# aask1357/hilcodec

Hardware: AMD Instinct MI355X
Metric: audio-seconds/sec (xRT) encode+RVQ+decode, 24 kHz batch=256 (higher is better)
Workload: dtype f32

## Files before the change

hilcodec_amd/csrc/resblock_kernel.h:

```cpp
#pragma once
#include "resblock_gemm.h"
#include "stream_gemm.h"

namespace {

struct Cols {
  long b;
  int t;
  int t_in;
  unsigned boff;
  unsigned hoff;
  int head, tail;
};
static_assert(sizeof(Cols) == 32, "no padding");

template <int C, bool STREAM, bool SCARRY = false, int NB = 1, bool W8 = false, int DRU = 0, bool POST = false, bool SPEC0 = false>
__global__ __launch_bounds__((Cfg<C, STREAM, SCARRY, NB, W8, DRU, POST, SPEC0>::NT), (Cfg<C, STREAM, SCARRY, NB, W8, DRU, POST, SPEC0>::MINW)) void resblock_kernel(ResArgs a) {
  using K = Cfg<C, STREAM, SCARRY, NB, W8, DRU, POST, SPEC0>;
  constexpr int DR = K::DR, UR = K::UR;
  using Pipe = WeightPipe<K>;
  constexpr int CBW = K::CBW, NW = K::NW, NT = K::NT, RW = K::RW, RB = K::RB, XS = K::XS, TO = K::TO, RSTEP = K::RSTEP;
  __shared__ __attribute__((aligned(16))) float Xbuf[4 + C * XS];
  constexpr bool DW_RELOAD = NB > 1 && K::NARROW && (4 + C * XS + NB * C * DWS) * 4 > 156 * 1024;
  __shared__ __attribute__((aligned(16))) float DW[(DW_RELOAD ? 1 : NB) * C * DWS];
  constexpr bool DWIDE = DR == 5 || DR == 8;
  __shared__ __attribute__((aligned(16))) float DWD[(DR > 0 && !DWIDE) ? 2 * C * DDS : 4];
  __shared__ __attribute__((aligned(16))) float HS[(STREAM && !K::NARROW) ? 2 * C * 4 : 4];
  __shared__ __attribute__((aligned(16))) float PR[POST ? POST_CLASSES * K::NCOL : 4];
  static_assert(!POST || (K::RPI * K::NW == POST_CLASSES), "a row class of the closing conv = the rows one half-wave walks");
  __shared__ __attribute__((aligned(16))) float SEG[SPEC0 ? (STREAM ? 256 : 192) : 4];
  __shared__ __attribute__((aligned(16))) float SEGS[SPEC0 ? (STREAM ? 256 : 192) : 4];
  float* const X = Xbuf + 4;
  const int tid = threadIdx.x, lane = tid & 63;
  const int wave = __builtin_amdgcn_readfirstlane(tid >> 6);
  constexpr int NCB = K::NCOL / 32;
  const int colblk = wave % NCB;
  const int wclass = wave / NCB;
  const int rowblk0 = wclass * CBW;
#if defined(HILC_DEBUG_WAVE_STAMPS)
  constexpr int WS_MAXB = 48;
  unsigned long long* ws_base = nullptr;
  int ws_k = 0;
#define STAMP(i) do { } while (0)
#define lds_barrier() do {                                                                                          \
    const unsigned long long t0_ = __builtin_amdgcn_s_memtime();                                                   \
    asm volatile("s_waitcnt lgkmcnt(0)" ::: "memory");                                                             \
    const unsigned long long t1_ = __builtin_amdgcn_s_memtime();                                                   \
    asm volatile("s_waitcnt lgkmcnt(0)\n\ts_barrier" ::: "memory");                                                 \
    const unsigned long long t2_ = __builtin_amdgcn_s_memtime();                                                   \
    if (ws_base != nullptr && lane == 0 && ws_k < WS_MAXB - 1) {                                                   \
      ws_base[ws_k * 3] = t0_; ws_base[ws_k * 3 + 1] = t1_; ws_base[ws_k * 3 + 2] = t2_;                           \
    }                                                                                                              \
    ++ws_k;                                                                                                        \
  } while (0)
#elif defined(HILC_DEBUG_STAMPS)
#define STAMP(i) do { if (a.dbg && tid == 0) a.dbg[stamp_tile * 8 + (i)] = __builtin_amdgcn_s_memtime(); } while (0)
  long stamp_tile = blockIdx.x;
#else
#define STAMP(i) do { } while (0)
#endif
  const int T = a.T;
  const int nblk = NB == 1 ? 1 : a.nblk;
  auto load_taps = [&](const ResBlk& bq, float* dst) {
    if constexpr (DW_RELOAD && !STREAM) {
      constexpr int NE = C * DWS;
      static_assert(NE % NT == 0, "whole rounds");
#pragma unroll
      for (int i = 0; i < NE / NT; ++i) {
        const int e = tid + i * NT;
        const int m = e / DWS, j = e - m * DWS;
        const float* src = j < 5 ? bq.dw1_w + (m * 5 + j) : (j == 5 ? bq.dw1_b + m : (j < 11 ? bq.dw2_w + (m * 5 + (j - 6)) : bq.dw2_b + m));
        dst[e] = *src;
      }
    } else if constexpr (DW_RELOAD) {
      constexpr int NE = C * DWS;
      static_assert(NE % NT == 0, "whole rounds");
#pragma unroll 3
      for (int i = 0; i < NE / NT; ++i) {
        const int e = tid + i * NT;
        const int m = e / DWS, j = e - m * DWS;
        const float* src = j < 5 ? bq.dw1_w + (m * 5 + j) : (j == 5 ? bq.dw1_b + m : (j < 11 ? bq.dw2_w + (m * 5 + (j - 6)) : bq.dw2_b + m));
        dst[e] = *src;
      }
    }
  };
  if constexpr (!DW_RELOAD) {
    constexpr int RND = (C + NT - 1) / NT;
    if constexpr (NB == 1 && STREAM) {
      const ResBlk& bq = a.blk[0];
#pragma unroll
      for (int it = 0; it < RND; ++it) {
        const int m = tid + it * NT;
        const int mc = (C % NT == 0 || m < C) ? m : C - 1;
#pragma unroll
        for (int w4 = 0; w4 < DWS / 4; ++w4) {
          float t4[4];
#pragma unroll
          for (int e = 0; e < 4; ++e) {
            const int j = 4 * w4 + e;
            t4[e] = j < 5 ? bq.dw1_w[mc * 5 + j] : (j == 5 ? bq.dw1_b[mc] : (j < 11 ? bq.dw2_w[mc * 5 + (j - 6)] : bq.dw2_b[mc]));
          }
          if (C % NT == 0 || m < C) *reinterpret_cast<f32x4*>(&DW[m * DWS + 4 * w4]) = f32x4{t4[0], t4[1], t4[2], t4[3]};
          __builtin_amdgcn_sched_barrier(0);
        }
      }
    } else {
    float tv[NB][RND][DWS];
#pragma unroll
    for (int q = 0; q < NB; ++q) {
      if (q < nblk) {
        const ResBlk& bq = a.blk[q];
#pragma unroll
        for (int it = 0; it < RND; ++it) {
          const int m = tid + it * NT;
          const int mc = (C % NT == 0 || m < C) ? m : C - 1;
#pragma unroll
          for (int j = 0; j < 5; ++j) tv[q][it][j] = bq.dw1_w[mc * 5 + j];
          tv[q][it][5] = bq.dw1_b[mc];
#pragma unroll
          for (int j = 0; j < 5; ++j) tv[q][it][6 + j] = bq.dw2_w[mc * 5 + j];
          tv[q][it][11] = bq.dw2_b[mc];
        }
      }
    }
#pragma unroll
    for (int q = 0; q < NB; ++q) {
      if (q < nblk) {
#pragma unroll
        for (int it = 0; it < RND; ++it) {
          const int m = tid + it * NT;
          if (C % NT == 0 || m < C) {
#pragma unroll
            for (int w4 = 0; w4 < DWS / 4; ++w4)
              *reinterpret_cast<f32x4*>(&DW[(q * C + m) * DWS + 4 * w4]) =
                  f32x4{tv[q][it][4 * w4], tv[q][it][4 * w4 + 1], tv[q][it][4 * w4 + 2], tv[q][it][4 * w4 + 3]};
          }
        }
      }
    }
    }
  }
  if constexpr (DR > 0 && !DWIDE) {
    constexpr int RND = (2 * C + NT - 1) / NT;
    float tw[RND][2 * DR + 1];
#pragma unroll
    for (int it = 0; it < RND; ++it) {
      const int m = tid + it * NT;
      const int mc = ((2 * C) % NT == 0 || m < 2 * C) ? m : 2 * C - 1;
#pragma unroll
      for (int j = 0; j < 2 * DR; ++j) tw[it][j] = a.dn.dw_w[mc * 2 * DR + j];
      tw[it][2 * DR] = a.dn.dw_b[mc];
    }
#pragma unroll
    for (int it = 0; it < RND; ++it) {
      const int m = tid + it * NT;
      if ((2 * C) % NT == 0 || m < 2 * C) {
#pragma unroll
        for (int j = 0; j < DDS; ++j) DWD[m * DDS + j] = j < 2 * DR ? tw[it][j] : (j == 8 ? tw[it][2 * DR] : 0.f);
      }
    }
  }
  if (tid < 4) Xbuf[tid] = 0.f;
  const int rsub = wave * K::RPI + (K::RPI > 1 ? lane / (K::NCOL / 4) : 0);
  const int c4 = (lane & (K::NCOL / 4 - 1)) * 4;
  [[maybe_unused]] const unsigned row_b = (unsigned)T * 4u;
  [[maybe_unused]] const bool one_head = STREAM && !K::NARROW && T >= K::NCOL;

  auto columns_of = [&](long tile) -> Cols {
    Cols s;
    s.boff = 0; s.hoff = 0; s.head = false; s.tail = false;
    if constexpr (STREAM) {
      const int flat = (int)tile * TO - K::HALO + c4;
      s.t_in = flat >= 0 && flat < a.B * T;
      const unsigned ub = s.t_in ? __umulhi((unsigned)flat, a.div_magic) >> a.div_shift : 0u;
      s.b = ub;
      s.t = s.t_in ? flat - (int)ub * T : 0;
      s.boff = (ub * (unsigned)(C * T) + (unsigned)s.t) * 4u;
      s.hoff = ub * (unsigned)(C * 4);
      s.head = s.t_in && s.t == 0;
      s.tail = s.t_in && c4 >= K::HALO && s.t == T - 4;
    } else {
      s.b = tile / a.tiles;
      s.t = (int)(tile - s.b * a.tiles) * TO + c4;
      s.t_in = s.t >= 0 && s.t < T;
    }
    return s;
  };
  auto xrow = [&](const Cols& s, int m) -> const f32x4* {
    if constexpr (STREAM)
      return reinterpret_cast<const f32x4*>(reinterpret_cast<const char*>(a.x) + (s.boff + (unsigned)m * row_b));
    else
      return reinterpret_cast<const f32x4*>(a.x + s.b * (long)C * T + (long)m * T + (s.t_in ? s.t : 0));
  };
  auto yrow = [&](const Cols& s, int m) -> f32x4* {
    if constexpr (STREAM)
      return reinterpret_cast<f32x4*>(reinterpret_cast<char*>(a.y) + (s.boff + (unsigned)m * row_b));
    else
      return reinterpret_cast<f32x4*>(a.y + s.b * (long)C * T + (long)m * T + s.t);
  };

  [[maybe_unused]] const float* hb0 = a.x;
  [[maybe_unused]] const float* hb1 = a.x;
  [[maybe_unused]] bool hv0 = false, hv1 = false;
  [[maybe_unused]] int blk_off = 0;
  Cols cs;
  const bool lane0 = c4 == 0, lane_last = c4 == K::NCOL - 4;
  auto prev_base = [&](int which) -> lptr_t {
    if constexpr (!K::CARRYMODE) return (lptr_t)(X + rsub * XS + c4 - 4);
    else return lane0 ? (lptr_t)(X + rsub * XS + K::NCOL + which * 4 + blk_off) : (lptr_t)(X + rsub * XS + c4 - 4);
  };
  auto prevs_of = [&](lptr_t pb, int m0, int which, f32x4 (&prev)[K::RB]) {
    if constexpr (!STREAM) {
#pragma unroll
      for (int i = 0; i < K::RB; ++i) prev[i] = *(lvec_t)(pb + i * RSTEP * XS);
    } else {
      bool staged = false;
      if constexpr (!K::NARROW) staged = one_head;
      if (staged) {
#pragma unroll
        for (int i = 0; i < K::RB; ++i) {
          const lptr_t pa = cs.head ? (lptr_t)(HS + (which * C + m0 + RSTEP * i) * 4) : pb + i * RSTEP * XS;
          prev[i] = *(lvec_t)pa;
        }
      } else {
        f32x4 hv[K::RB];
#pragma unroll
        for (int i = 0; i < K::RB; ++i)
          hv[i] = *reinterpret_cast<const f32x4*>((which ? hb1 : hb0) + ((which ? hv1 : hv0) ? cs.hoff + (unsigned)(m0 + RSTEP * i) * 4u : 0u));
#pragma unroll
        for (int i = 0; i < K::RB; ++i) {
          const f32x4 own = *(lvec_t)(pb + i * RSTEP * XS);
#pragma unroll
          for (int e = 0; e < 4; ++e) prev[i][e] = cs.head ? ((which ? hv1 : hv0) ? hv[i][e] : 0.f) : own[e];
        }
      }
    }
  };
  auto carry_out = [&](lptr_t xp, int which, const f32x4 (&cur)[K::RB]) {
    if constexpr (K::CARRYMODE) {
      if (lane_last) {
#pragma unroll
        for (int i = 0; i < K::RB; ++i) *(lvec_t)(xp + i * RSTEP * XS + 4 + which * 4 + blk_off) = cur[i];
      }
    }
  };

  float touch = 0.f;
  constexpr int LPR = K::NCOL / 32;
#ifdef HILC_RES_NO_UTOUCH
  constexpr bool UTOUCH = false;
#else
  constexpr bool UTOUCH = !STREAM && UR > 0 && !K::NARROW && (K::NCOL / (UR > 0 ? UR : 1)) % 32 == 0;
#endif
  constexpr int LPRU = UTOUCH ? K::NCOL / UR / 32 : 1;
  constexpr int NTOUCH = STREAM ? 1 : (UTOUCH ? (2 * C * LPRU + NT - 1) / NT : (C * LPR + NT - 1) / NT);
  float tv[NTOUCH];
#pragma unroll
  for (int i = 0; i < NTOUCH; ++i) tv[i] = 0.f;
  __shared__ long s_next;
  long run0 = blockIdx.x, run1 = a.total_tiles;
  long tile = blockIdx.x;
  if constexpr (K::CARRYMODE) {
    if (a.classes > 1) {
      const unsigned P = gridDim.x / (unsigned)a.classes, u = blockIdx.x % P, c = blockIdx.x / P;
      const long s0 = (long)u * a.total_tiles / P, len = (long)(u + 1) * a.total_tiles / P - s0;
      run0 = s0 + ((len * (long)a.cum[c]) >> 16);
      run1 = s0 + ((len * (long)a.cum[c + 1]) >> 16);
    } else if (a.run_tiles > 0) {
      run0 = (long)blockIdx.x * a.run_tiles;
      run1 = run0 + a.run_tiles < a.total_tiles ? run0 + a.run_tiles : a.total_tiles;
    } else {
      run0 = (long)blockIdx.x * a.total_tiles / gridDim.x;
      run1 = ((long)blockIdx.x + 1) * a.total_tiles / gridDim.x;
    }
    const bool mid = STREAM ? (run0 * TO) % T != 0 : run0 % a.tiles != 0;
    tile = (mid && run0 < run1) ? run0 - 1 : run0;
  }
  cs = columns_of(tile < run1 ? tile : 0);
  f32x4 xr[RW];
  if (UR == 0 && !SPEC0 && tile < run1) {
#pragma unroll
    for (int i = 0; i < RW; ++i) xr[i] = *xrow(cs, rsub + RSTEP * i);
  }
// ... 54 lines not shown
              const long row = (long)cs.b * (2 * C) + k;
              const float* xi = up.xin + (cs.t_in ? row * Tin + q0 : 0);
              xc[i] = xi[0];
              const float* pp = has_prev ? xi - 1 : (up.hist != nullptr && cs.t_in ? up.hist + row : xi);
              xq[i] = pp[0];
              if constexpr (UR == 2) {
                xn[i] = xi[cs.t_in ? 1 : 0];
                wa[i] = *reinterpret_cast<const f32x4*>(up.tr_w + k * 4);
              } else if constexpr (UEXP) {
                xn[i] = xi[has_next ? 1 : 0];
                const float* tw = up.tr_w + ((long)k * UR + p0) * 8;
                wa[i] = *reinterpret_cast<const f32x4*>(tw);
                wb[i] = *reinterpret_cast<const f32x4*>(tw + 4);
              } else {
                wa[i] = *reinterpret_cast<const f32x4*>(up.tr_w + k * (2 * UR) + p0);
                wb[i] = *reinterpret_cast<const f32x4*>(up.tr_w + k * (2 * UR) + UR + p0);
              }
            }
#pragma unroll
            for (int i = 0; i < UB; ++i) {
              const float a1 = prologue(xc[i], up.in_scale, 1);
              const float a0 = has_prev ? prologue(xq[i], up.in_scale, 1) : (up.hist != nullptr ? xq[i] : 0.f);
              f32x4 u;
              float a_last = a1;
              if constexpr (UR == 2) {
                const float a2 = prologue(xn[i], up.in_scale, 1);
                u[0] = fmaf(wa[i].x, a1, wa[i].z * a0);
                u[1] = fmaf(wa[i].y, a1, wa[i].w * a0);
                u[2] = fmaf(wa[i].x, a2, wa[i].z * a1);
                u[3] = fmaf(wa[i].y, a2, wa[i].w * a1);
                a_last = a2;
              } else if constexpr (UEXP) {
                const float a2 = has_next ? prologue(xn[i], up.in_scale, 1) : 0.f;
#pragma unroll
                for (int e = 0; e < 4; ++e) {
                  const bool nx = p0 + e >= UR;
                  u[e] = fmaf(wa[i][e], nx ? a2 : a1, wb[i][e] * (nx ? a1 : a0));
                }
                a_last = p0 + 3 >= UR ? a2 : a1;
              } else {
#pragma unroll
                for (int e = 0; e < 4; ++e) u[e] = fmaf(wa[i][e], a1, wb[i][e] * a0);
              }
              *(lvec_t)(xp + i * RSTEP * XS) = zero_unless(cs.t_in, u);
              if constexpr (STREAM) {
                if (cs.tail && !warm && up.hist_out != nullptr)
                  up.hist_out[(long)cs.b * (2 * C) + h * C + rsub + RSTEP * (i0 + i)] = a_last;
              }
            }
            xp += UB * RSTEP * XS;
            asm volatile("" : "+v"(xp));
            __builtin_amdgcn_sched_barrier(0);
          }
        }
        Pipe wp;
        wp.prefetch(wu, lane);
        lds_barrier();
        if constexpr (K::NARROW) gemm_phase_rolled<K, false>(wu, X, acc, wp, colblk, lane);
        else gemm_phase<K, false>(wu, X, acc, wp, colblk, lane);
        lds_barrier();
      }
      acc_to_x<K>(acc, X, rowblk0, colblk, lane);
      lds_barrier();
      {
        lptr_t xp = (lptr_t)(X + rsub * XS + c4);
#pragma unroll
        for (int i = 0; i < RW; ++i) {
          const float bv = up.bias != nullptr ? up.bias[rsub + RSTEP * i] : 0.f;
          f32x4 v = *(lvec_t)(xp + i * RSTEP * XS);
#pragma unroll
          for (int e = 0; e < 4; ++e) v[e] = up.bias != nullptr ? __fadd_rn(v[e], bv) : v[e];
          xr[i] = v;
        }
      }
      lds_barrier();
    }
    if constexpr (SPEC0) {
      const ResSpec0& sp = a.spec;
      constexpr int N = 64, NBIN = 33, SROWS = 40, KP0 = 4, DEPTH0 = 2;
      [[maybe_unused]] int split = K::NCOL;
      if constexpr (STREAM) {
        const int F0 = (int)tile * TO;
        const unsigned bA = __umulhi((unsigned)F0, a.div_magic) >> a.div_shift;
        const int tA0 = F0 - (int)bA * T;
        const int nxt = T - tA0;
        split = nxt < K::NCOL ? nxt : K::NCOL;
        const int lenA = (N - 1) + split;
        for (int i = tid; i < 2 * (N - 1) + K::NCOL; i += NT) {
          const bool second = i >= lenA;
          const unsigned b = bA + (second ? 1u : 0u);
          const int t = second ? i - lenA - (N - 1) : tA0 - (N - 1) + i;
          float v = 0.f;
          if (b < (unsigned)a.B) {
            if (t >= 0) v = sp.wav[(long)b * T + t];
            else if (sp.hist != nullptr && t >= -sp.hist_len) v = sp.hist[(long)b * sp.hist_len + sp.hist_len + t];
          }
          SEG[i] = v;
          SEGS[i] = v * sp.pre_in_scale;
        }
        for (int i = tid; i < (SROWS - NBIN) * 128; i += NT) X[(NBIN + (i >> 7)) * XS + (i & 127)] = 0.f;
      } else {
      const int f0 = cs.t - c4;
      {
        const int s0 = f0 - (N - 1);
        const float* wb = sp.wav + cs.b * (long)T;
        for (int i = tid; i < 127 + N; i += NT) {
          const int t = s0 + i;
          const float v = (t >= 0 && t < T) ? wb[t] : 0.f;
          SEG[i] = v;
          SEGS[i] = v * sp.pre_in_scale;
        }
        for (int i = tid; i < (SROWS - NBIN) * 128; i += NT) X[(NBIN + (i >> 7)) * XS + (i & 127)] = 0.f;
      }
      }
      lds_barrier();
      const int kh = lane >> 5, col = colblk * 32 + (lane & 31);
      const int colx = col + ((STREAM && col >= split) ? N - 1 : 0);
      f32x16 acc[CBW];
      {
        int off[8];
#pragma unroll
        for (int p = 0; p < 8; ++p) off[p] = colx + 2 * p + kh;
        auto bop = [&](int P) -> float { return SEG[off[P & 7] + 16 * (P >> 3)]; };
        stream_gemm<CBW, KP0, DEPTH0, N / 2 / KP0>(sp.dft, acc, lane, bop);
      }
      float nyq_im = 0.f;
#pragma unroll 8
      for (int k = 0; k < N; ++k) nyq_im = fmaf(sp.nyq[k], SEG[colx + k], nyq_im);
      const SpecFinish finish = SpecFinish::make(sp.mean, sp.stdv, sp.normalize);
#pragma unroll
      for (int i = 0; i < CBW; ++i) {
#pragma unroll
        for (int r = 0; r < 16; r += 2) {
          const int row = i * 32 + acc_row(r, lane);
          if (i == 0 && r == 0) {
            if (kh == 0) {
              X[0 * XS + col] = finish(acc[0][0], 0.f);
              X[(N / 2) * XS + col] = finish(acc[0][1], nyq_im);
            } else {
              X[(row >> 1) * XS + col] = finish(acc[0][0], acc[0][1]);
            }
          } else {
            X[(row >> 1) * XS + col] = finish(acc[i][r], acc[i][r + 1]);
          }
        }
      }
      lds_barrier();
      {
        const float* sl = X + kh * XS + col;
        auto bop = [&](int P) -> float { return sl[2 * P * XS]; };
        stream_gemm<CBW, KP0, DEPTH0, SROWS / 2 / KP0>(sp.pw, acc, lane, bop);
      }
      lds_barrier();
      acc_to_x<K>(acc, X, rowblk0, colblk, lane);
      lds_barrier();
      {
        lptr_t xp = (lptr_t)(X + rsub * XS + c4);
        float sm[8];
        const int c4x = c4 + ((STREAM && c4 >= split) ? N - 1 : 0);
#pragma unroll
        for (int j = 0; j < 8; ++j) sm[j] = SEGS[c4x + j + N - 5];
#pragma unroll
        for (int i = 0; i < RW; ++i) {
          const int m = rsub + RSTEP * i;
          const float bv = sp.bias != nullptr ? sp.bias[m] : 0.f;
          const float pb = sp.pre_b != nullptr ? sp.pre_b[m] : 0.f;
          float w5[5];
#pragma unroll
          for (int j = 0; j < 5; ++j) w5[j] = sp.pre_w[m * 5 + j];
          f32x4 v = *(lvec_t)(xp + i * RSTEP * XS);
#pragma unroll
          for (int e = 0; e < 4; ++e) {
            float acc5 = 0.f;
#pragma unroll
            for (int j = 0; j < 5; ++j) acc5 = fmaf(w5[j], sm[e + j], acc5);
            const float rr = sp.pre_b != nullptr ? __fadd_rn(acc5, pb) : acc5;
            float t = v[e];
            if (sp.bias != nullptr) t = __fadd_rn(t, bv);
            t = __fmul_rn(t, sp.out_scale);
            v[e] = __fadd_rn(t, rr);
          }
          xr[i] = v;
          if (i % 2 == 1) __builtin_amdgcn_sched_barrier(0);
        }
      }
      lds_barrier();
    }
#pragma nounroll
    for (int blk = 0; blk < nblk; ++blk) {
    const ResBlk& bp = a.blk[NB == 1 ? 0 : blk];
    const bool final_blk = NB == 1 || blk == nblk - 1;
    const bool last_blk = DR == 0 && !POST && final_blk;
    [[maybe_unused]] const bool post_blk = POST && final_blk;
    Cols cn = cs;
    bool have_next = false;
    if constexpr (NB > 1) blk_off = 8 * blk;
    const float* const DWb = DW + ((NB == 1 || DW_RELOAD) ? 0 : blk * C * DWS);
    if constexpr (DW_RELOAD) load_taps(bp, DW);
    if constexpr (STREAM) {
      hb0 = bp.hist1 != nullptr ? bp.hist1 : a.x;
      hb1 = bp.hist2 != nullptr ? bp.hist2 : a.x;
      hv0 = bp.hist1 != nullptr;
      hv1 = bp.hist2 != nullptr;
    }
    const float* w1t = bp.w1t + (long)wclass * (C * C / K::RH);
    const float* w2t = bp.w2t + (long)wclass * (C * C / K::RH);
    asm volatile("" : "+s"(w1t), "+s"(w2t));
    [[maybe_unused]] f32x4 hstage[(STREAM && !K::NARROW) ? (2 * C + NT - 1) / NT : 1];
    [[maybe_unused]] bool stage_hs = false;
    if constexpr (STREAM && !K::NARROW) {
      if (one_head) {
        const int first = (int)tile * TO - K::HALO, last = first + K::NCOL - 1;
        const unsigned bh = __umulhi((unsigned)last, a.div_magic) >> a.div_shift;
        const int hcol = (int)bh * T;
        stage_hs = hcol >= first && (int)bh < a.B;
        if (stage_hs) {
#pragma unroll
          for (int q = 0; q < (2 * C + NT - 1) / NT; ++q) {
            const int e = tid + q * NT;
            const int which = e >= C ? 1 : 0, m = e - which * C;
            f32x4 v = {0.f, 0.f, 0.f, 0.f};
            if (e < 2 * C && (which ? hv1 : hv0)) v = *reinterpret_cast<const f32x4*>((which ? hb1 : hb0) + bh * (unsigned)(C * 4) + (unsigned)m * 4u);
            hstage[q] = v;
          }
        }
      }
    }
    Pipe wp;
    wp.prefetch(w1t, lane);
    {
      lptr_t xp = (lptr_t)(X + rsub * XS + c4);
#pragma unroll
      for (int i0 = 0; i0 < RW; i0 += RB) {
#pragma unroll
        for (int i = 0; i < RB; ++i)
          *(lvec_t)(xp + i * RSTEP * XS) = prologue4v(zero_unless(cs.t_in, xr[i0 + i]), bp.pre_scale, 1);
        xp += RB * RSTEP * XS;
        asm volatile("" : "+v"(xp));
      }
    }
#pragma unroll
    for (int i = 0; i < NTOUCH; ++i) touch += tv[i];
    if constexpr (STREAM && !K::NARROW) {
      if (stage_hs) {
#pragma unroll
        for (int q = 0; q < (2 * C + NT - 1) / NT; ++q) {
          const int e = tid + q * NT;
          if (e < 2 * C) *reinterpret_cast<f32x4*>(&HS[e * 4]) = hstage[q];
        }
      }
    }
    lds_barrier();
    STAMP(1);
    if (TICKETS && a.sched != nullptr) next_tile = s_next;

    f32x16 acc[CBW];
    if constexpr (K::NARROW) gemm_phase_rolled<K>(w1t, X, acc, wp, colblk, lane);
    else gemm_phase<K>(w1t, X, acc, wp, colblk, lane);
    lds_barrier();
    STAMP(2);
    acc_to_x<K>(acc, X, rowblk0, colblk, lane);
    lds_barrier();
    STAMP(3);

    wp.prefetch(w2t, lane);
    lptr_t xp3 = (lptr_t)(X + rsub * XS + c4);
    lptr_t pb3 = prev_base(0);
#pragma unroll
    for (int i0 = 0; i0 < RW; i0 += RB) {
// ... 163 lines not shown
      lptr_t xq = (lptr_t)(X + rsub * XS + c4);
      lptr_t pq = lane0 ? (lptr_t)(X + rsub * XS + PSLOT) : (lptr_t)(X + rsub * XS + c4 - 4);
      const float* wq = a.post.w + rsub * 5;
      [[maybe_unused]] bool any_head = false;
      [[maybe_unused]] const float* hq = a.post.w;
      [[maybe_unused]] float* hqo = nullptr;
      [[maybe_unused]] bool qtail = false;
      if constexpr (STREAM) {
        const int first = (int)tile * TO, last = first + K::NCOL - 1;
        const unsigned bl = __umulhi((unsigned)last, a.div_magic) >> a.div_shift;
        any_head = (int)bl * T >= first || first % T == 0;
        if (a.post.hist != nullptr) hq = a.post.hist + cs.hoff + rsub * 4;
        qtail = cs.tail && !warm && a.post.hist_out != nullptr;
        if (a.post.hist_out != nullptr) hqo = a.post.hist_out + cs.hoff + rsub * 4;
      }
#pragma nounroll
      for (int i0 = 0; i0 < RW; i0 += RB) {
        f32x4 cur[RB], prev[RB];
        float w[RB][5];
#pragma unroll
        for (int i = 0; i < RB; ++i) {
          cur[i] = *(lvec_t)(xq + i * RSTEP * XS);
          prev[i] = *(lvec_t)(pq + i * RSTEP * XS);
#pragma unroll
          for (int j = 0; j < 5; ++j) w[i][j] = wq[i * RSTEP * 5 + j];
        }
        wq += RB * RSTEP * 5;
        if constexpr (STREAM) {
          if (any_head) {
            f32x4 hv[RB];
#pragma unroll
            for (int i = 0; i < RB; ++i)
              hv[i] = a.post.hist != nullptr ? *reinterpret_cast<const f32x4*>(hq + i * RSTEP * 4) : f32x4{0.f, 0.f, 0.f, 0.f};
#pragma unroll
            for (int i = 0; i < RB; ++i)
#pragma unroll
              for (int e = 0; e < 4; ++e) prev[i][e] = cs.head ? hv[i][e] : prev[i][e];
          }
          if (qtail) {
#pragma unroll
            for (int i = 0; i < RB; ++i) *reinterpret_cast<f32x4*>(hqo + i * RSTEP * 4) = cur[i];
          }
          hq += a.post.hist != nullptr ? RB * RSTEP * 4 : 0;
          hqo += RB * RSTEP * 4;
        }
        if (lane_last) {
#pragma unroll
          for (int i = 0; i < RB; ++i) *(lvec_t)(xq + i * RSTEP * XS + 4 + 8 * NB) = cur[i];
        }
#pragma unroll
        for (int i = 0; i < RB; ++i) {
          const float v[8] = {prev[i].x, prev[i].y, prev[i].z, prev[i].w, cur[i].x, cur[i].y, cur[i].z, cur[i].w};
#pragma unroll
          for (int e = 0; e < 4; ++e)
#pragma unroll
            for (int j = 0; j < 5; ++j) part[e] = fmaf(w[i][j], v[e + j], part[e]);
        }
        xq += RB * RSTEP * XS;
        pq += RB * RSTEP * XS;
        asm volatile("" : "+v"(xq), "+v"(pq));
        __builtin_amdgcn_sched_barrier(0);
      }
      *reinterpret_cast<f32x4*>(&PR[rsub * K::NCOL + c4]) = f32x4{part[0], part[1], part[2], part[3]};
      lds_barrier();
      if (tid < K::NCOL) {
        float sacc = PR[tid];
#pragma unroll
        for (int q = 1; q < POST_CLASSES; ++q) sacc = __fadd_rn(sacc, PR[q * K::NCOL + tid]);
        if (a.post.bias != nullptr) sacc = __fadd_rn(sacc, a.post.bias[0]);
        sacc = __fmul_rn(sacc, a.post.out_scale);
        if (a.post.do_tanh) sacc = tanhf(sacc);
        if constexpr (STREAM) {
          const long flat = (long)tile * TO + tid;
          if (!warm && flat < (long)a.B * T) a.post.wav[flat] = sacc;
        } else {
          const int t = cs.t - c4 + tid;
          if (!warm && t < T) a.post.wav[cs.b * (long)T + t] = sacc;
        }
      }
      cs = cn;
    }
    if constexpr (DR > 0) {
      const ResDown& dn = a.dn;
      const bool have_next = next_tile < run1;
      const Cols cn = columns_of(have_next ? next_tile : tile);
      const float* wd0 = dn.w_lo + (long)wclass * (C * C / K::RH);
      const float* wd1 = dn.w_hi + (long)wclass * (C * C / K::RH);
      asm volatile("" : "+s"(wd0), "+s"(wd1));
      Pipe wp;
      wp.prefetch(wd0, lane);
      auto d0 = [&]() {
        lptr_t xp = (lptr_t)(X + rsub * XS + c4);
#pragma unroll
        for (int i0 = 0; i0 < RW; i0 += RB) {
#pragma unroll
          for (int i = 0; i < RB; ++i)
            *(lvec_t)(xp + i * RSTEP * XS) = prologue4v(zero_unless(cs.t_in, xr[i0 + i]), dn.in_scale, 1);
          xp += RB * RSTEP * XS;
          asm volatile("" : "+v"(xp));
        }
      };
      d0();
      if (!DWIDE && !SPEC0 && have_next) {
#pragma unroll
        for (int i = 0; i < RW; ++i) xr[i] = *xrow(cn, rsub + RSTEP * i);
      }
      lds_barrier();
      f32x16 acc0[CBW];
      [[maybe_unused]] f32x16 acc1[DWIDE ? 1 : CBW];
      if constexpr (K::NARROW) gemm_phase_rolled<K>(wd0, X, acc0, wp, colblk, lane);
      else gemm_phase<K>(wd0, X, acc0, wp, colblk, lane);
      if constexpr (!DWIDE) {
        wp.prefetch(wd1, lane);
        if constexpr (K::NARROW) gemm_phase_rolled<K>(wd1, X, acc1, wp, colblk, lane);
        else gemm_phase<K>(wd1, X, acc1, wp, colblk, lane);
      }
      const bool out_ok = !warm && (STREAM ? cs.t_in : cs.t < T);
      [[maybe_unused]] const bool out_ok_tile = !warm;
      const int To = T / DR;
#pragma unroll
      for (int h = 0; h < 2; ++h) {
        if constexpr (DWIDE) {
          if (h == 1) {
            lds_barrier();
            wp.prefetch(wd1, lane);
            d0();
            if (have_next) {
#pragma unroll
              for (int i = 0; i < RW; ++i) xr[i] = *xrow(cn, rsub + RSTEP * i);
            }
            lds_barrier();
            gemm_phase_rolled<K>(wd1, X, acc0, wp, colblk, lane);
          }
        }
        lds_barrier();
        if constexpr (DWIDE) acc_to_x<K>(acc0, X, rowblk0, colblk, lane);
        else acc_to_x<K>(h ? acc1 : acc0, X, rowblk0, colblk, lane);
        lds_barrier();
        if constexpr (DWIDE) {
          constexpr int DC = K::DCAR;
          constexpr int DOFF = K::NCOL + 8 * NB;
          constexpr bool SLOTS = K::CARRYMODE;
          const int jl = c4 >> 2;
          const int t0 = STREAM ? (int)tile * TO : cs.t - c4;
          const int o = t0 / DR + jl;
          const int base = o * DR - DR - t0;
          [[maybe_unused]] unsigned sb = 0;
          int os = o;
          if constexpr (STREAM) {
            const bool in = o < a.B * To;
            sb = in ? __umulhi((unsigned)(o * DR), a.div_magic) >> a.div_shift : 0u;
            os = in ? o - (int)sb * To : 1;
          }
          [[maybe_unused]] const bool dhead = STREAM && os == 0;
          const bool act = out_ok_tile && (STREAM ? o < a.B * To : o < To) && o * DR + DR - 1 < t0 + K::NCOL;
          [[maybe_unused]] const int slot = DOFF + DC * h + DC;
          lptr_t rowp = (lptr_t)(X + rsub * XS);
          const float* wrow = dn.dw_w + (long)(h * C + rsub) * (2 * DR);
          const float* brow = dn.dw_b + (h * C + rsub);
          float wn[2 * DR], bn;
          [[maybe_unused]] float hn[STREAM ? DR : 1];
          [[maybe_unused]] const float* hrow = dn.dw_w;
          [[maybe_unused]] float* horow = nullptr;
          [[maybe_unused]] const bool use_hist = STREAM && dn.hist != nullptr;
          if constexpr (STREAM) {
            if (use_hist) hrow = dn.hist + ((long)sb * (2 * C) + h * C + rsub) * DR;
            if (dn.hist_out != nullptr) horow = dn.hist_out + ((long)cs.b * (2 * C) + h * C + rsub) * DR;
          }
          [[maybe_unused]] const bool dtail = STREAM && cs.tail && !warm && dn.hist_out != nullptr;
          auto taps_of = [&](const float* wr, const float* br) {
            if constexpr (DR == 8) {
#pragma unroll
              for (int q = 0; q < 4; ++q) {
                const f32x4 w4 = *reinterpret_cast<const f32x4*>(wr + 4 * q);
#pragma unroll
                for (int e = 0; e < 4; ++e) wn[4 * q + e] = w4[e];
              }
            } else {
#pragma unroll
              for (int q = 0; q < DR; ++q) {
                const f32x2 w2 = *reinterpret_cast<const f32x2*>(wr + 2 * q);
                wn[2 * q] = w2.x; wn[2 * q + 1] = w2.y;
              }
            }
            bn = br[0];
            if constexpr (STREAM) {
              if (use_hist) {
                if constexpr (DR == 8) {
#pragma unroll
                  for (int q = 0; q < 2; ++q) {
                    const f32x4 h4 = *reinterpret_cast<const f32x4*>(hrow + 4 * q);
#pragma unroll
                    for (int e = 0; e < 4; ++e) hn[4 * q + e] = h4[e];
                  }
                } else {
#pragma unroll
                  for (int j = 0; j < DR; ++j) hn[j] = hrow[j];
                }
              } else {
#pragma unroll
                for (int j = 0; j < DR; ++j) hn[j] = 0.f;
              }
            }
          };
          taps_of(wrow, brow);
          long yo = STREAM ? ((long)sb * (2 * C) + h * C + rsub) * (long)To + os : ((long)cs.b * (2 * C) + h * C + rsub) * (long)To + o;
#pragma nounroll
          for (int i0 = 0; i0 < RW; ++i0) {
            float v[2 * DR], w[2 * DR];
#pragma unroll
            for (int j = 0; j < 2 * DR; ++j) w[j] = wn[j];
            const float bb = bn;
            [[maybe_unused]] float hc[STREAM ? DR : 1];
            if constexpr (STREAM) {
#pragma unroll
              for (int j = 0; j < DR; ++j) hc[j] = hn[j];
            }
            wrow += RSTEP * (2 * DR);
            brow += RSTEP;
            if constexpr (STREAM) hrow += use_hist ? RSTEP * DR : 0;
            if (i0 + 1 < RW) taps_of(wrow, brow);
            if constexpr (DR == 8) {
#pragma unroll
              for (int q = 0; q < 4; ++q) {
                const int col = base + 4 * q;
                const f32x4 x4 = *(lvec_t)(rowp + (col >= 0 ? col : (SLOTS ? slot + col : 0)));
#pragma unroll
                for (int e = 0; e < 4; ++e) v[4 * q + e] = x4[e];
              }
            } else {
#pragma unroll
              for (int j = 0; j < 2 * DR; ++j) {
                const int col = base + j;
                v[j] = *(rowp + (col >= 0 ? col : (SLOTS ? slot + col : 0)));
              }
            }
            if constexpr (STREAM) {
#pragma unroll
              for (int j = 0; j < DR; ++j) v[j] = dhead ? hc[j] : v[j];
            }
            const f32x4 keep = *(lvec_t)(rowp + c4);
            if constexpr (STREAM) {
              const f32x4 before = *(lvec_t)(rowp + (c4 >= 4 ? c4 - 4 : 0));
              if (dtail) {
                if constexpr (DR == 8) {
                  *reinterpret_cast<f32x4*>(horow) = before;
                  *reinterpret_cast<f32x4*>(horow + 4) = keep;
                } else {
                  horow[0] = before.w; horow[1] = keep.x; horow[2] = keep.y; horow[3] = keep.z; horow[4] = keep.w;
                }
              }
              horow += RSTEP * DR;
            }
            if constexpr (SLOTS) {
              if (c4 >= K::NCOL - DC)
                *(lvec_t)(rowp + DOFF + DC * h + (c4 - (K::NCOL - DC))) = keep;
            }
            float s0 = 0.f;
#pragma unroll
            for (int j = 0; j < 2 * DR; ++j) s0 = fmaf(w[j], v[j], s0);
            s0 = __fadd_rn(s0, bb);
            if (act) dn.y[yo] = dn.res != nullptr ? __fadd_rn(s0, dn.res[yo]) : s0;
            yo += (long)RSTEP * To;
            rowp += RSTEP * XS;
          }
        } else {
        lptr_t xpd = (lptr_t)(X + rsub * XS + c4);
        lptr_t pbd = lane0 ? (lptr_t)(X + rsub * XS + K::NCOL + 8 * NB + 4 * h) : (lptr_t)(X + rsub * XS + c4 - 4);
#pragma unroll
        for (int i0 = 0; i0 < RW; i0 += RB) {
          f32x4 cur[RB], prev[RB], wa[RB], wb[RB];
          float bb[RB];
#pragma unroll
          for (int i = 0; i < RB; ++i) {
            const int m = h * C + rsub + RSTEP * (i0 + i);
            cur[i] = *(lvec_t)(xpd + i * RSTEP * XS);
            prev[i] = *(lvec_t)(pbd + i * RSTEP * XS);
            wa[i] = *reinterpret_cast<const f32x4*>(&DWD[m * DDS]);
            if constexpr (DR == 4) wb[i] = *reinterpret_cast<const f32x4*>(&DWD[m * DDS + 4]);
            bb[i] = DWD[m * DDS + 8];
          }
          if constexpr (STREAM) {
            const unsigned hro = (unsigned)cs.b * (unsigned)(2 * C * DR) + (unsigned)(h * C + rsub + RSTEP * i0) * DR;
#pragma unroll
            for (int i = 0; i < RB; ++i) {
              f32x4 hv = {0.f, 0.f, 0.f, 0.f};
              if (dn.hist != nullptr) {
                const float* hp = dn.hist + (cs.t_in ? hro + (unsigned)(RSTEP * i * DR) : 0u);
                if constexpr (DR == 4) hv = *reinterpret_cast<const f32x4*>(hp);
                else { const f32x2 h2 = *reinterpret_cast<const f32x2*>(hp); hv = f32x4{0.f, 0.f, h2.x, h2.y}; }
              }
#pragma unroll
              for (int e = 0; e < 4; ++e) prev[i][e] = cs.head ? hv[e] : prev[i][e];
            }
          }
          if (lane_last) {
#pragma unroll
            for (int i = 0; i < RB; ++i) *(lvec_t)(xpd + i * RSTEP * XS + 4 + 8 * NB + 4 * h) = cur[i];
          }
          if constexpr (STREAM) {
            if (cs.tail && !warm && dn.hist_out != nullptr) {
              const unsigned hro = (unsigned)cs.b * (unsigned)(2 * C * DR) + (unsigned)(h * C + rsub + RSTEP * i0) * DR;
#pragma unroll
              for (int i = 0; i < RB; ++i) {
                float* hp = dn.hist_out + hro + (unsigned)(RSTEP * i * DR);
                if constexpr (DR == 4) *reinterpret_cast<f32x4*>(hp) = cur[i];
                else *reinterpret_cast<f32x2*>(hp) = f32x2{cur[i].z, cur[i].w};
              }
            }
          }
#pragma unroll
          for (int i = 0; i < RB; ++i) {
            const int m = h * C + rsub + RSTEP * (i0 + i);
            const long yo = ((long)cs.b * (2 * C) + m) * (long)To + (cs.t_in ? cs.t / DR : 0);
            if constexpr (DR == 4) {
              const float v[8] = {prev[i].x, prev[i].y, prev[i].z, prev[i].w, cur[i].x, cur[i].y, cur[i].z, cur[i].w};
              const float w[8] = {wa[i].x, wa[i].y, wa[i].z, wa[i].w, wb[i].x, wb[i].y, wb[i].z, wb[i].w};
              float s0 = 0.f;
#pragma unroll
              for (int j = 0; j < 8; ++j) s0 = fmaf(w[j], v[j], s0);
              s0 = __fadd_rn(s0, bb[i]);
              if (out_ok) dn.y[yo] = dn.res != nullptr ? __fadd_rn(s0, dn.res[yo]) : s0;
            } else {
              const float v[6] = {prev[i].z, prev[i].w, cur[i].x, cur[i].y, cur[i].z, cur[i].w};
              const float w[4] = {wa[i].x, wa[i].y, wa[i].z, wa[i].w};
              f32x2 o2;
#pragma unroll
              for (int e = 0; e < 2; ++e) {
                float s0 = 0.f;
#pragma unroll
                for (int j = 0; j < 4; ++j) s0 = fmaf(w[j], v[2 * e + j], s0);
                o2[e] = __fadd_rn(s0, bb[i]);
              }
              if (out_ok) {
                if (dn.res != nullptr) {
                  const f32x2 r2 = *reinterpret_cast<const f32x2*>(dn.res + yo);
                  o2[0] = __fadd_rn(o2[0], r2.x);
                  o2[1] = __fadd_rn(o2[1], r2.y);
                }
                *reinterpret_cast<f32x2*>(dn.y + yo) = o2;
              }
            }
          }
          xpd += RB * RSTEP * XS;
          pbd += RB * RSTEP * XS;
          asm volatile("" : "+v"(xpd), "+v"(pbd));
          __builtin_amdgcn_sched_barrier(0);
        }
        }
      }
      lds_barrier();
      cs = cn;
    }
    tile = next_tile;
  }
  if (!K::CARRYMODE && K::NW == 4 && a.sched != nullptr && tid == 0) {
    if (atomicAdd(a.sched + 1, 1) == (int)gridDim.x - 1) {
      a.sched[0] = 0;
      a.sched[1] = 0;
    }
  }
  if (touch == 1.2345678e-30f) a.y[0] = touch;
#if defined(HILC_DEBUG_WAVE_STAMPS)
  if (ws_base != nullptr && lane == 0) ws_base[(WS_MAXB - 1) * 3 + 1] = (unsigned long long)ws_k;
#undef lds_barrier
#endif
#undef STAMP
}

}
```

hilcodec_amd/csrc/stream_gemm.h:

```cpp
#pragma once
#include "gemm_core.h"

namespace hilc {

typedef const __attribute__((address_space(1))) float* sg_gptr_t;
typedef const __attribute__((address_space(1))) f32x4* sg_gvec_t;

template <int CB, int KP, int DEPTH, int NSETS, class BOp>
__device__ __forceinline__ void stream_gemm(const float* __restrict__ wt, f32x16 (&acc)[CB], int lane, BOp bop) {
  constexpr int WPS = KP * CB / 4;
  float a[DEPTH][KP][CB];
  float b[DEPTH][KP];
  auto load_word = [&](sg_gptr_t wset, int slot, int q) {
    const f32x4 v = *(sg_gvec_t)(wset + q * 256 + lane * 4);
#pragma unroll
    for (int e = 0; e < 4; ++e) a[slot][(q * 4 + e) / CB][(q * 4 + e) % CB] = v[e];
  };
#pragma unroll
  for (int d = 0; d < DEPTH - 1; ++d) {
    if (d < NSETS) {
#pragma unroll
      for (int q = 0; q < WPS; ++q) load_word((sg_gptr_t)(wt + d * WPS * 256), d, q);
#pragma unroll
      for (int j = 0; j < KP; ++j) b[d][j] = bop(d * KP + j);
    }
  }
  const float* wn = wt + (DEPTH - 1) * WPS * 256;
  constexpr int LD_EVERY = KP * CB / WPS;
#pragma unroll
  for (int s = 0; s < NSETS; ++s) {
    const int cur = s % DEPTH, nxt = (s + DEPTH - 1) % DEPTH;
    const int sn = s + DEPTH - 1;
    const bool more = sn < NSETS;
#pragma unroll
    for (int j = 0; j < KP; ++j) {
      if (more) b[nxt][j] = bop(sn * KP + j);
#pragma unroll
      for (int i = 0; i < CB; ++i) {
        const int n = j * CB + i;
        if (more && n % LD_EVERY == 0) load_word((sg_gptr_t)wn, nxt, n / LD_EVERY);
        if (s == 0 && j == 0) {
#pragma unroll
          for (int r = 0; r < 16; ++r) acc[i][r] = 0.f;
        }
        acc[i] = __builtin_amdgcn_mfma_f32_32x32x2f32(a[cur][j][i], b[cur][j], acc[i], 0, 0, 0);
      }
    }
    if (more) {
      wn += WPS * 256;
      asm volatile("" : "+s"(wn));
    }
#pragma unroll
    for (int i = 0; i < CB; ++i) asm volatile("" : "+v"(acc[i]) :: "memory");
  }
}

}
```

Before: 3511.

## Overlap stage-0 spectrogram prologue work and trim its barriers and global loads

```diff
diff --git a/hilcodec_amd/csrc/resblock_kernel.h b/hilcodec_amd/csrc/resblock_kernel.h
--- a/hilcodec_amd/csrc/resblock_kernel.h
+++ b/hilcodec_amd/csrc/resblock_kernel.h
@@ -30,6 +30,11 @@
   static_assert(!POST || (K::RPI * K::NW == POST_CLASSES), "a row class of the closing conv = the rows one half-wave walks");
   __shared__ __attribute__((aligned(16))) float SEG[SPEC0 ? (STREAM ? 256 : 192) : 4];
   __shared__ __attribute__((aligned(16))) float SEGS[SPEC0 ? (STREAM ? 256 : 192) : 4];
+  constexpr int SPS = 8;
+  __shared__ __attribute__((aligned(16))) float NYQ[SPEC0 ? 64 : 4];
+  __shared__ __attribute__((aligned(16))) float SPW[SPEC0 ? C * SPS : 4];
+  static_assert(!SPEC0 || sizeof(Xbuf) + sizeof(DW) + sizeof(DWD) + sizeof(HS) + sizeof(PR) + sizeof(SEG) + sizeof(SEGS) + sizeof(NYQ) + sizeof(SPW) + 64 <= 80 * 1024,
+                "stage 0: two workgroups per CU");
   float* const X = Xbuf + 4;
   const int tid = threadIdx.x, lane = tid & 63;
   const int wave = __builtin_amdgcn_readfirstlane(tid >> 6);
@@ -42,6 +47,7 @@
   unsigned long long* ws_base = nullptr;
   int ws_k = 0;
 #define STAMP(i) do { } while (0)
+#define STAMP_SD(i) do { } while (0)
 #define lds_barrier() do {                                                                                          \
     const unsigned long long t0_ = __builtin_amdgcn_s_memtime();                                                   \
     asm volatile("s_waitcnt lgkmcnt(0)" ::: "memory");                                                             \
@@ -54,10 +60,18 @@
     ++ws_k;                                                                                                        \
   } while (0)
 #elif defined(HILC_DEBUG_STAMPS)
-#define STAMP(i) do { if (a.dbg && tid == 0) a.dbg[stamp_tile * 8 + (i)] = __builtin_amdgcn_s_memtime(); } while (0)
+#if defined(HILC_DEBUG_STAMPS_SD)
+  constexpr int STAMP_SLOTS = 32;
+#define STAMP_SD(i) STAMP(i)
+#else
+  constexpr int STAMP_SLOTS = 8;
+#define STAMP_SD(i) do { } while (0)
+#endif
+#define STAMP(i) do { if (a.dbg && tid == 0) a.dbg[stamp_tile * STAMP_SLOTS + (i)] = __builtin_amdgcn_s_memtime(); } while (0)
   long stamp_tile = blockIdx.x;
 #else
 #define STAMP(i) do { } while (0)
+#define STAMP_SD(i) do { } while (0)
 #endif
   const int T = a.T;
   const int nblk = NB == 1 ? 1 : a.nblk;
@@ -158,6 +172,20 @@
 #pragma unroll
         for (int j = 0; j < DDS; ++j) DWD[m * DDS + j] = j < 2 * DR ? tw[it][j] : (j == 8 ? tw[it][2 * DR] : 0.f);
       }
+    }
+  }
+  if constexpr (SPEC0) {
+    static_assert(NT >= C && C == 64, "one row of the first conv, one word of the Nyquist row per thread");
+    if (tid < C) {
+      const ResSpec0& sp = a.spec;
+      float w5[5];
+#pragma unroll
+      for (int j = 0; j < 5; ++j) w5[j] = sp.pre_w[tid * 5 + j];
+      const float pb = sp.pre_b != nullptr ? sp.pre_b[tid] : 0.f;
+      const float bv = sp.bias != nullptr ? sp.bias[tid] : 0.f;
+      NYQ[tid] = sp.nyq[tid];
+      *reinterpret_cast<f32x4*>(&SPW[tid * SPS]) = f32x4{w5[0], w5[1], w5[2], w5[3]};
+      *reinterpret_cast<f32x4*>(&SPW[tid * SPS + 4]) = f32x4{w5[4], pb, bv, 0.f};
     }
   }
   if (tid < 4) Xbuf[tid] = 0.f;
@@ -199,6 +227,33 @@
       return reinterpret_cast<f32x4*>(a.y + s.b * (long)C * T + (long)m * T + s.t);
   };
 
+  constexpr int SEGN = STREAM ? 2 * 63 + K::NCOL : 63 + K::NCOL;
+  static_assert(!SPEC0 || SEGN <= NT, "one segment word per thread");
+  [[maybe_unused]] auto seg_fetch = [&](long tl) -> float {
+    const ResSpec0& sp = a.spec;
+    float v = 0.f;
+    if constexpr (STREAM) {
+      const int F0 = (int)tl * TO;
+      const unsigned bA = __umulhi((unsigned)F0, a.div_magic) >> a.div_shift;
+      const int tA0 = F0 - (int)bA * T;
+      const int nxt = T - tA0;
+      const int lenA = 63 + (nxt < K::NCOL ? nxt : K::NCOL);
+      const bool second = tid >= lenA;
+      const unsigned b = bA + (second ? 1u : 0u);
+      const int t = second ? tid - lenA - 63 : tA0 - 63 + tid;
+      if (tid < SEGN && b < (unsigned)a.B) {
+        if (t >= 0) v = sp.wav[(long)b * T + t];
+        else if (sp.hist != nullptr && t >= -sp.hist_len) v = sp.hist[(long)b * sp.hist_len + sp.hist_len + t];
+      }
+    } else {
+      const long b = tl / a.tiles;
+      const int t = (int)(tl - b * a.tiles) * TO - 63 + tid;
+      if (tid < SEGN && t >= 0 && t < T) v = sp.wav[b * (long)T + t];
+    }
+    return v;
+  };
+  [[maybe_unused]] float segv = 0.f;
+  [[maybe_unused]] bool seg_ready = false;
   [[maybe_unused]] const float* hb0 = a.x;
   [[maybe_unused]] const float* hb1 = a.x;
   [[maybe_unused]] bool hv0 = false, hv1 = false;
@@ -419,51 +474,42 @@
       if constexpr (STREAM) {
         const int F0 = (int)tile * TO;
         const unsigned bA = __umulhi((unsigned)F0, a.div_magic) >> a.div_shift;
-        const int tA0 = F0 - (int)bA * T;
-        const int nxt = T - tA0;
+        const int nxt = T - (F0 - (int)bA * T);
         split = nxt < K::NCOL ? nxt : K::NCOL;
-        const int lenA = (N - 1) + split;
-        for (int i = tid; i < 2 * (N - 1) + K::NCOL; i += NT) {
-          const bool second = i >= lenA;
-          const unsigned b = bA + (second ? 1u : 0u);
-          const int t = second ? i - lenA - (N - 1) : tA0 - (N - 1) + i;
-          float v = 0.f;
-          if (b < (unsigned)a.B) {
-            if (t >= 0) v = sp.wav[(long)b * T + t];
-            else if (sp.hist != nullptr && t >= -sp.hist_len) v = sp.hist[(long)b * sp.hist_len + sp.hist_len + t];
-          }
-          SEG[i] = v;
-          SEGS[i] = v * sp.pre_in_scale;
-        }
-        for (int i = tid; i < (SROWS - NBIN) * 128; i += NT) X[(NBIN + (i >> 7)) * XS + (i & 127)] = 0.f;
-      } else {
-      const int f0 = cs.t - c4;
-      {
-        const int s0 = f0 - (N - 1);
-        const float* wb = sp.wav + cs.b * (long)T;
-        for (int i = tid; i < 127 + N; i += NT) {
-          const int t = s0 + i;
-          const float v = (t >= 0 && t < T) ? wb[t] : 0.f;
-          SEG[i] = v;
-          SEGS[i] = v * sp.pre_in_scale;
-        }
-        for (int i = tid; i < (SROWS - NBIN) * 128; i += NT) X[(NBIN + (i >> 7)) * XS + (i & 127)] = 0.f;
-      }
-      }
+      }
+      if (!seg_ready) segv = seg_fetch(tile);
+      if (tid < SEGN) {
+        SEG[tid] = segv;
+        SEGS[tid] = segv * sp.pre_in_scale;
+      }
+      for (int i = tid; i < (SROWS - NBIN) * 128; i += NT) X[(NBIN + (i >> 7)) * XS + (i & 127)] = 0.f;
       lds_barrier();
+      STAMP_SD(8);
       const int kh = lane >> 5, col = colblk * 32 + (lane & 31);
       const int colx = col + ((STREAM && col >= split) ? N - 1 : 0);
       f32x16 acc[CBW];
+      float nyq_im = 0.f;
       {
         int off[8];
 #pragma unroll
         for (int p = 0; p < 8; ++p) off[p] = colx + 2 * p + kh;
         auto bop = [&](int P) -> float { return SEG[off[P & 7] + 16 * (P >> 3)]; };
-        stream_gemm<CBW, KP0, DEPTH0, N / 2 / KP0>(sp.dft, acc, lane, bop);
-      }
-      float nyq_im = 0.f;
-#pragma unroll 8
-      for (int k = 0; k < N; ++k) nyq_im = fmaf(sp.nyq[k], SEG[colx + k], nyq_im);
+        constexpr int NSET = N / 2 / KP0;
+        static_assert(NSET * 8 == N, "eight links per register set");
+        float nq[8], sg[8];
+        auto nyq_load = [&](int s8) {
+#pragma unroll
+          for (int e = 0; e < 8; ++e) { nq[e] = NYQ[8 * s8 + e]; sg[e] = SEG[colx + 8 * s8 + e]; }
+        };
+        nyq_load(0);
+        auto nyq_links = [&](int s8) {
+#pragma unroll
+          for (int e = 0; e < 8; ++e) nyq_im = fmaf(nq[e], sg[e], nyq_im);
+          if (s8 + 1 < NSET) nyq_load(s8 + 1);
+        };
+        stream_gemm<CBW, KP0, DEPTH0, NSET>(sp.dft, acc, lane, bop, nyq_links);
+      }
+      STAMP_SD(9);
       const SpecFinish finish = SpecFinish::make(sp.mean, sp.stdv, sp.normalize);
 #pragma unroll
       for (int i = 0; i < CBW; ++i) {
@@ -482,15 +528,16 @@
           }
         }
       }
-      lds_barrier();
+      STAMP_SD(10);
       {
         const float* sl = X + kh * XS + col;
         auto bop = [&](int P) -> float { return sl[2 * P * XS]; };
         stream_gemm<CBW, KP0, DEPTH0, SROWS / 2 / KP0>(sp.pw, acc, lane, bop);
       }
-      lds_barrier();
+      STAMP_SD(11);
       acc_to_x<K>(acc, X, rowblk0, colblk, lane);
       lds_barrier();
+      STAMP_SD(12);
       {
         lptr_t xp = (lptr_t)(X + rsub * XS + c4);
         float sm[8];
@@ -500,11 +547,10 @@
 #pragma unroll
         for (int i = 0; i < RW; ++i) {
           const int m = rsub + RSTEP * i;
-          const float bv = sp.bias != nullptr ? sp.bias[m] : 0.f;
-          const float pb = sp.pre_b != nullptr ? sp.pre_b[m] : 0.f;
-          float w5[5];
-#pragma unroll
-          for (int j = 0; j < 5; ++j) w5[j] = sp.pre_w[m * 5 + j];
+          const f32x4 wa = *reinterpret_cast<const f32x4*>(&SPW[m * SPS]);
+          const f32x4 wb = *reinterpret_cast<const f32x4*>(&SPW[m * SPS + 4]);
+          const float w5[5] = {wa.x, wa.y, wa.z, wa.w, wb.x};
+          const float pb = wb.y, bv = wb.z;
           f32x4 v = *(lvec_t)(xp + i * RSTEP * XS);
 #pragma unroll
           for (int e = 0; e < 4; ++e) {
@@ -522,6 +568,7 @@
         }
       }
       lds_barrier();
+      STAMP_SD(13);
     }
 #pragma nounroll
     for (int blk = 0; blk < nblk; ++blk) {
@@ -851,11 +898,34 @@
     }
     if constexpr (DR > 0) {
       const ResDown& dn = a.dn;
+      STAMP_SD(16);
       const bool have_next = next_tile < run1;
       const Cols cn = columns_of(have_next ? next_tile : tile);
       const float* wd0 = dn.w_lo + (long)wclass * (C * C / K::RH);
       const float* wd1 = dn.w_hi + (long)wclass * (C * C / K::RH);
       asm volatile("" : "+s"(wd0), "+s"(wd1));
+      constexpr bool YWALK = SPEC0 && DR == 2;
+      constexpr bool RES_PRE = YWALK && !STREAM;
+      [[maybe_unused]] f32x2 rpre[2][RES_PRE ? RW : 1];
+      typedef const __attribute__((address_space(1))) f32x2* gvec2_t;
+      [[maybe_unused]] int rsub_d = rsub;
+      if constexpr (YWALK) asm volatile("" : "+v"(rsub_d));
+      [[maybe_unused]] const long yo_tile = ((long)cs.b * (2 * C)) * (long)(T / DR) + (cs.t_in ? cs.t / DR : 0);
+      [[maybe_unused]] auto res_fetch = [&](int h, f32x2 (&r)[RES_PRE ? RW : 1]) {
+        if (dn.res != nullptr && !warm && (STREAM ? cs.t_in : cs.t < T)) {
+          const float* rp = dn.res + yo_tile + (unsigned)(h * C + rsub_d) * (unsigned)(T / DR);
+#pragma unroll
+          for (int i = 0; i < (RES_PRE ? RW : 1); ++i) {
+            r[i] = *(gvec2_t)rp;
+            rp += (long)RSTEP * (long)(T / DR);
+            asm volatile("" : "+v"(rp));
+          }
+        }
+      };
+      if constexpr (RES_PRE) {
+        res_fetch(0, rpre[0]);
+        res_fetch(1, rpre[1]);
+      }
       Pipe wp;
       wp.prefetch(wd0, lane);
       auto d0 = [&]() {
@@ -875,6 +945,7 @@
         for (int i = 0; i < RW; ++i) xr[i] = *xrow(cn, rsub + RSTEP * i);
       }
       lds_barrier();
+      STAMP_SD(17);
       f32x16 acc0[CBW];
       [[maybe_unused]] f32x16 acc1[DWIDE ? 1 : CBW];
       if constexpr (K::NARROW) gemm_phase_rolled<K>(wd0, X, acc0, wp, colblk, lane);
@@ -884,6 +955,11 @@
         if constexpr (K::NARROW) gemm_phase_rolled<K>(wd1, X, acc1, wp, colblk, lane);
         else gemm_phase<K>(wd1, X, acc1, wp, colblk, lane);
       }
+      if constexpr (SPEC0) {
+        seg_ready = have_next;
+        if (have_next) segv = seg_fetch(next_tile);
+      }
+      STAMP_SD(18);
       const bool out_ok = !warm && (STREAM ? cs.t_in : cs.t < T);
       [[maybe_unused]] const bool out_ok_tile = !warm;
       const int To = T / DR;
@@ -906,6 +982,7 @@
         if constexpr (DWIDE) acc_to_x<K>(acc0, X, rowblk0, colblk, lane);
         else acc_to_x<K>(h ? acc1 : acc0, X, rowblk0, colblk, lane);
         lds_barrier();
+        STAMP_SD(19 + 2 * h);
         if constexpr (DWIDE) {
           constexpr int DC = K::DCAR;
           constexpr int DOFF = K::NCOL + 8 * NB;
@@ -1036,6 +1113,7 @@
         } else {
         lptr_t xpd = (lptr_t)(X + rsub * XS + c4);
         lptr_t pbd = lane0 ? (lptr_t)(X + rsub * XS + K::NCOL + 8 * NB + 4 * h) : (lptr_t)(X + rsub * XS + c4 - 4);
+        [[maybe_unused]] long yod = YWALK ? yo_tile + (unsigned)(h * C + rsub_d) * (unsigned)To : 0;
 #pragma unroll
         for (int i0 = 0; i0 < RW; i0 += RB) {
           f32x4 cur[RB], prev[RB], wa[RB], wb[RB];
@@ -1081,7 +1159,8 @@
 #pragma unroll
           for (int i = 0; i < RB; ++i) {
             const int m = h * C + rsub + RSTEP * (i0 + i);
-            const long yo = ((long)cs.b * (2 * C) + m) * (long)To + (cs.t_in ? cs.t / DR : 0);
+            long yo = yod;
+            if constexpr (!YWALK) yo = ((long)cs.b * (2 * C) + m) * (long)To + (cs.t_in ? cs.t / DR : 0);
             if constexpr (DR == 4) {
               const float v[8] = {prev[i].x, prev[i].y, prev[i].z, prev[i].w, cur[i].x, cur[i].y, cur[i].z, cur[i].w};
               const float w[8] = {wa[i].x, wa[i].y, wa[i].z, wa[i].w, wb[i].x, wb[i].y, wb[i].z, wb[i].w};
@@ -1103,12 +1182,18 @@
               }
               if (out_ok) {
                 if (dn.res != nullptr) {
-                  const f32x2 r2 = *reinterpret_cast<const f32x2*>(dn.res + yo);
+                  f32x2 r2;
+                  if constexpr (RES_PRE) r2 = rpre[h][i0 + i];
+                  else r2 = *reinterpret_cast<const f32x2*>(dn.res + yo);
                   o2[0] = __fadd_rn(o2[0], r2.x);
                   o2[1] = __fadd_rn(o2[1], r2.y);
                 }
                 *reinterpret_cast<f32x2*>(dn.y + yo) = o2;
               }
+              if constexpr (YWALK) {
+                yod += (long)RSTEP * (long)To;
+                asm volatile("" : "+v"(yod));
+              }
             }
           }
           xpd += RB * RSTEP * XS;
@@ -1117,8 +1202,10 @@
           __builtin_amdgcn_sched_barrier(0);
         }
         }
+        STAMP_SD(20 + 2 * h);
       }
       lds_barrier();
+      STAMP_SD(23);
       cs = cn;
     }
     tile = next_tile;
@@ -1135,6 +1222,7 @@
 #undef lds_barrier
 #endif
 #undef STAMP
+#undef STAMP_SD
 }
 
 }
diff --git a/hilcodec_amd/csrc/stream_gemm.h b/hilcodec_amd/csrc/stream_gemm.h
--- a/hilcodec_amd/csrc/stream_gemm.h
+++ b/hilcodec_amd/csrc/stream_gemm.h
@@ -6,8 +6,10 @@
 typedef const __attribute__((address_space(1))) float* sg_gptr_t;
 typedef const __attribute__((address_space(1))) f32x4* sg_gvec_t;
 
-template <int CB, int KP, int DEPTH, int NSETS, class BOp>
-__device__ __forceinline__ void stream_gemm(const float* __restrict__ wt, f32x16 (&acc)[CB], int lane, BOp bop) {
+struct NoSide { __device__ __forceinline__ void operator()(int) const {} };
+
+template <int CB, int KP, int DEPTH, int NSETS, class BOp, class Side = NoSide>
+__device__ __forceinline__ void stream_gemm(const float* __restrict__ wt, f32x16 (&acc)[CB], int lane, BOp bop, Side side = Side()) {
   constexpr int WPS = KP * CB / 4;
   float a[DEPTH][KP][CB];
   float b[DEPTH][KP];
@@ -46,6 +48,7 @@
         acc[i] = __builtin_amdgcn_mfma_f32_32x32x2f32(a[cur][j][i], b[cur][j], acc[i], 0, 0, 0);
       }
     }
+    side(s);
     if (more) {
       wn += WPS * 256;
       asm volatile("" : "+s"(wn));
```

Result: no change. 3515, median of 3 (+0.1%).
